# composewell/streamly-lz4

Hardware: AMD Instinct MI355X
Metric: GB/s uncompressed (compress+decompress), 64 KiB blocks, 1/2/4/8 GPU (higher is better)
Workload: dtype u8

## Files before the change

### streamly-lz4_amd/csrc/decode_par.hpp

```cpp
#pragma once

#include "decode_seq.hpp"

namespace lz4dev {

#define PAR_NODES 512
#ifndef PAR_ADAPT
#define PAR_ADAPT 1
#endif
#ifndef PAR_TAIL_ROUND
#define PAR_TAIL_ROUND 2
#endif
#ifndef PAR_ADAPT6
#define PAR_ADAPT6 416
#endif
#ifndef PAR_ADAPT10
#define PAR_ADAPT10 0
#endif
#define PAR_MAXNODES (PAR_ADAPT10 ? 640 : 512)
#ifndef PAR_SQ
#define PAR_SQ 3
#endif
#ifndef PAR_WIN
#define PAR_WIN 832
#endif
#ifndef PAR_RING
#define PAR_RING 5088
#endif
#ifndef PAR_HIST
#define PAR_HIST 1500
#endif
#ifndef PAR_BATCH_OUT
#define PAR_BATCH_OUT 1856
#endif
#ifndef PAR_FAR_WIDE
#define PAR_FAR_WIDE 0
#endif
#ifndef PAR_RANK
#define PAR_RANK 1
#endif
#ifndef PAR_PRIO
#define PAR_PRIO 0x33
#endif
#ifndef PAR_WAVES
#define PAR_WAVES 5
#endif
#ifndef PAR_WAVES_MAIN
#define PAR_WAVES_MAIN 8
#endif

#define PAR_JUMP_BYTES (2 * (PAR_MAXNODES + 8))
#define PAR_JUMP_OFS ((PAR_RING + 32 - PAR_JUMP_BYTES) & ~15)
#define PAR_WIN_BYTES (PAR_WIN + 32)
#define PAR_WIN_OFS (PAR_JUMP_OFS - PAR_WIN_BYTES)
#define PAR_FREE_OFS ((PAR_RING - PAR_BATCH_OUT - 32 + 15) & ~15)
struct __attribute__((aligned(16))) ParLds {
    uint8_t ring[PAR_RING + 32];
    __device__ __forceinline__ uint16_t *jump() { return (uint16_t *)&ring[PAR_JUMP_OFS]; }
    __device__ __forceinline__ uint8_t *win() { return &ring[PAR_WIN_OFS]; }
};
#define PAR_END (2 * PAR_NODES)
#ifndef PAR_LDS_LIMIT
#define PAR_LDS_LIMIT 5120
#endif
static_assert(sizeof(ParLds) <= PAR_LDS_LIMIT, "ParLds above four 1280-byte LDS granules: 24 waves per CU or fewer instead of 28");
static_assert(PAR_WIN_BYTES % 16 == 0 && PAR_JUMP_OFS % 16 == 0 && PAR_WIN_OFS % 16 == 0,
              "the table, its 16-byte rank records and the window's 16-byte slots are aligned");
static_assert(PAR_WIN_OFS >= 0 && PAR_WIN_OFS + PAR_WIN_BYTES <= PAR_JUMP_OFS && PAR_JUMP_OFS + PAR_JUMP_BYTES <= PAR_RING + 32,
              "the window and the table lie inside ring[], one behind the other");
static_assert(PAR_JUMP_BYTES + PAR_WIN_BYTES <= PAR_BATCH_OUT + 64 && PAR_WIN_OFS >= PAR_FREE_OFS && PAR_JUMP_OFS >= PAR_FREE_OFS,
              "the overlays lie on ring bytes that hold no output from a batch's end to the next batch's first store (the no-slide bound)");
#define PAR_WIN_LANES (PAR_WIN / 16)
static_assert(PAR_WIN % 16 == 0 && PAR_WIN_LANES <= LZ4_WAVE, "the window is 16 bytes per lane");
static_assert(PAR_MAXNODES + 288 <= PAR_WIN + 32, "a plain sequence that starts at the last node, and the reads behind it, stay in the window");
static_assert(PAR_HIST + 30 + PAR_BATCH_OUT + 32 <= PAR_RING, "a batch fits the ring right after a slide");

typedef uint64_t par_u64u __attribute__((aligned(1)));
typedef uint32_t par_u32u __attribute__((aligned(1)));
typedef uint16_t par_u16u __attribute__((aligned(1)));

typedef uint32_t par_v4 __attribute__((ext_vector_type(4)));
typedef par_v4 par_v4u __attribute__((aligned(1)));

__device__ __forceinline__ uint32_t lds_u32_any(const uint8_t *base4, uint32_t addr)
{
    const uint32_t *p = (const uint32_t *)(base4 + (addr & ~3u));
    return __builtin_amdgcn_alignbyte(p[1], p[0], addr & 3u);
}
__device__ __forceinline__ uint64_t lds_u64_any(const uint8_t *base4, uint32_t addr)
{
    const uint32_t *p = (const uint32_t *)(base4 + (addr & ~3u));
    const uint32_t d0 = p[0], d1 = p[1], d2 = p[2];
    const uint32_t sh = addr & 3u;
    return ((uint64_t)__builtin_amdgcn_alignbyte(d2, d1, sh) << 32) | __builtin_amdgcn_alignbyte(d1, d0, sh);
}

__device__ __forceinline__ int par_bperm(int v, int srcLane)
{
    return __builtin_amdgcn_ds_bpermute(srcLane << 2, v);
}

template <int D>
__device__ __forceinline__ int par_row_shr(int v)
{
    return __builtin_amdgcn_update_dpp(0, v, 0x110 | D, 0xf, 0xf, true);
}

__device__ __forceinline__ int par_scan_incl(int x)
{
    x += __builtin_amdgcn_update_dpp(0, x, 0x111, 0xf, 0xf, true);
    x += __builtin_amdgcn_update_dpp(0, x, 0x112, 0xf, 0xf, true);
    x += __builtin_amdgcn_update_dpp(0, x, 0x114, 0xf, 0xf, true);
    x += __builtin_amdgcn_update_dpp(0, x, 0x118, 0xf, 0xf, true);
    x += __builtin_amdgcn_update_dpp(0, x, 0x142, 0xa, 0xf, false);
    x += __builtin_amdgcn_update_dpp(0, x, 0x143, 0xc, 0xf, false);
    return x;
}

__device__ __forceinline__ uint4 par_fetch_window_edge(const uint8_t *q, const uint8_t *bufLo, const uint8_t *bufHi)
{
    uint32_t E[8] = {0u, 0u, 0u, 0u, 0u, 0u, 0u, 0u};
    uint32_t m = 0;
    if (q + 16 > bufLo && q < bufHi) {
        const uint8_t *qc = (q < bufLo) ? bufLo : bufHi - 16;
        par_v4 v;
        __builtin_memcpy(&v, as_global(qc), 16);
        const bool below = q < bufLo;
        const uint32_t d = (uint32_t)(below ? bufLo - q : q - qc);
        m = below ? 16u - d : d;
        E[0] = below ? 0u : v.x; E[1] = below ? 0u : v.y; E[2] = below ? 0u : v.z; E[3] = below ? 0u : v.w;
        E[4] = below ? v.x : 0u; E[5] = below ? v.y : 0u; E[6] = below ? v.z : 0u; E[7] = below ? v.w : 0u;
    }
    if (m & 8u) { for (int i = 0; i < 6; i++) E[i] = E[i + 2]; }
    if (m & 4u) { for (int i = 0; i < 5; i++) E[i] = E[i + 1]; }
    uint32_t w[4];
    for (int i = 0; i < 4; i++) w[i] = __builtin_amdgcn_alignbyte(E[i + 1], E[i], m & 3u);
    return make_uint4(w[0], w[1], w[2], w[3]);
}

enum { PS_BATCHES, PS_SEQS, PS_ROUNDS, PS_MATCH_ITERS, PS_LIT_ITERS, PS_HANDOVERS, PS_SLIDES, PS_FULL, PS_FAR,
       PS_T_WINDOW, PS_T_SPEC, PS_T_CHAIN, PS_T_DECODE, PS_T_LIT, PS_T_NEED, PS_T_MATCH, PS_T_FLUSH, PS_T_SEQ, PS_COUNT };

template <bool STATS, bool DICT, bool TOL = false, bool LIST = false, bool PARTIAL = false>
__device__ int decode_block_par(const uint8_t *src, int srcLen, uint8_t *dst, int cap, const uint8_t *dict,
                                uint32_t dictLen, const uint8_t *bufLo, const uint8_t *bufHi, ParLds &L,
                                unsigned long long *stats, TolCtx *tol = nullptr, const uint8_t *list = nullptr,
                                int listLen = 0)
{
    int li = 0;
    int nodesPerLane = 8;
    uint32_t sc[PS_COUNT];
    uint32_t tmark = 0;
    if (STATS) {
#pragma unroll
        for (int i = 0; i < PS_COUNT; i++) sc[i] = 0;
        tmark = (uint32_t)__builtin_amdgcn_readfirstlane((int)(uint32_t)__builtin_amdgcn_s_memtime());
    }
    auto lap = [&](int which) {
        if (STATS) {
            const uint32_t now = (uint32_t)__builtin_amdgcn_readfirstlane((int)(uint32_t)__builtin_amdgcn_s_memtime());
            sc[which] += now - tmark;
            tmark = now;
        }
    };
    auto publish = [&]() {
        if (STATS && lane_id() == 0) {
#pragma unroll
            for (int i = 0; i < PS_COUNT; i++) atomicAdd(&stats[i], (unsigned long long)sc[i]);
        }
    };
    static_assert(!PARTIAL || (!DICT && !TOL), "the partial mode has no dictionary");
    if (DICT) {
        auto up = [](const uint8_t *p) -> const uint8_t * { return (const uint8_t *)(uintptr_t)uni64((int64_t)(uintptr_t)p); };
        src = up(src); dst = (uint8_t *)up(dst); dict = up(dict); bufLo = up(bufLo); bufHi = up(bufHi); list = up(list);
        srcLen = uni(srcLen); cap = uni(cap); dictLen = (uint32_t)uni((int)dictLen); listLen = uni(listLen);
    }
    if (cap < 128 || srcLen < 64) return decode_block_seq<TOL, PARTIAL>(src, srcLen, dst, cap, dict, dictLen, bufLo, bufHi, tol);
    if (!DICT) { dict = nullptr; dictLen = 0; }
    const uint8_t *dictEnd = DICT ? dict + dictLen : dst;
    const int dictLo = DICT ? -(int)min(dictLen, 65535u) : 0;

    int lane;
    asm volatile("v_mbcnt_lo_u32_b32 %0, -1, 0\n\tv_mbcnt_hi_u32_b32 %0, -1, %0" : "=v"(lane));
    const int iend = srcLen;
    const uint32_t A = (uint32_t)((uintptr_t)dst & 15);
    int ip = 0, op = 0;
    int ringBase = 0;
    int flushed = 0;
    SeqState st;

    auto fresh = [](int v) -> int { asm volatile("" : "+v"(v)); return v; };
    constexpr bool MAIN = !DICT && !TOL && !PARTIAL;
    auto win_lane = [&]() -> int { return (PAR_WIN_LANES < LZ4_WAVE) ? min(lane, PAR_WIN_LANES - 1) : lane; };
    auto fetch_window = [&](uintptr_t base) -> uint4 {
        const uint8_t *q = (const uint8_t *)(base + 16u * (uint32_t)win_lane());
        if (__builtin_expect(q >= bufLo && q + 16 <= bufHi, 1)) {
            const par_v4 v = *as_global((const par_v4 *)q);
            return make_uint4(v.x, v.y, v.z, v.w);
        }
        return par_fetch_window_edge(q, bufLo, bufHi);
    };

#ifndef PAR_FLUSH
#define PAR_FLUSH 64
#endif
    const uint32_t AF = (uint32_t)((uintptr_t)dst & (PAR_FLUSH - 1));
    auto flush = [&](int upto, bool final) {
        wave_fence();
        int f = flushed;
        const int mis = (int)((AF + (uint32_t)f) & (PAR_FLUSH - 1));
        if (mis) {
            const int head = PAR_FLUSH - mis;
            if (upto - f >= head) {
                if (lane < head) dst[f + lane] = L.ring[f - ringBase + (int)A + lane];
                f += head;
            } else if (!final) {
                return;
            }
        }
        if (((AF + (uint32_t)f) & (PAR_FLUSH - 1)) == 0) {
            const int n16 = final ? (upto - f) >> 4 : ((upto - f) / PAR_FLUSH) * (PAR_FLUSH / 16);
            for (int c = fresh(lane); c < n16; c += LZ4_WAVE) {
                const uint4 v = *(const uint4 *)&L.ring[f - ringBase + (int)A + 16 * c];
                *(uint4 *)(dst + f + 16 * c) = v;
            }
            f += n16 << 4;
        }
        if (final) {
            for (int x = f + lane; x < upto; x += LZ4_WAVE) dst[x] = L.ring[x - ringBase + (int)A];
            f = upto;
        }
        flushed = f;
        wave_fence();
    };

    uintptr_t wbase = (uintptr_t)src & ~(uintptr_t)15;
    uint4 wnext = fetch_window(wbase);
    bool winStale = true;
    const uint8_t *jumpB = (const uint8_t *)L.jump();

    for (;;) {
        while (iend - ip >= 64 && cap - op >= 128) {
            lap(PS_T_FLUSH);

            const uint8_t *gp = src + ip;
            const uintptr_t abase = (uintptr_t)gp & ~(uintptr_t)15;
            const int wofs = (int)((uintptr_t)gp - abase);
            const int ipW0 = ip - wofs;
            const int iendW = iend - ipW0;
            const int inLim = min(iendW - 32, PAR_WIN);
            if (abase != wbase) { wbase = abase; wnext = fetch_window(abase); winStale = true; }
            if (winStale) {
                *(uint4 *)&L.win()[16 * win_lane()] = wnext;
                winStale = false;
                wave_fence();
            }
            lap(PS_T_WINDOW);

            uint32_t c2, absorb;
            bool fromList = false;
            if (LIST && li < listLen) {
                fromList = true;
                absorb = 2u * (uint32_t)max(inLim, 0);
                const int k = li + lane;
                const uint32_t d = (k < listLen) ? (uint32_t)as_global(list)[k] : 0u;
                const uint64_t zm = __ballot(d == 0u);
                const int known = zm ? (int)__builtin_ctzll(zm) : LZ4_WAVE - 1;
                const int incl0 = par_scan_incl((int)d);
                c2 = (lane <= known) ? 2u * (uint32_t)(wofs + incl0 - (int)d) : absorb;
                c2 = min(c2, absorb);
            } else {
            const int &laneId = lane;
            auto parse_square = [&](auto NC) {
                constexpr int NL = decltype(NC)::value;
                static_assert(NL % 2 == 0 && NL * LZ4_WAVE <= PAR_MAXNODES, "pairs of nodes, table size");
                const int lane = MAIN ? fresh(laneId) : laneId;
                uint32_t J[NL];
                absorb = 2u * ((uint32_t)min(inLim, NL * LZ4_WAVE - 1) + 1u);
                {
                    typedef unsigned short par_h2 __attribute__((ext_vector_type(2)));
                    uint32_t w0, w1, w2;
                    if (NL == 8) {
                        const uint64_t lo = *(const uint64_t *)&L.win()[8 * lane];
                        w0 = (uint32_t)lo; w1 = (uint32_t)(lo >> 32);
                        w2 = (uint32_t)__builtin_amdgcn_update_dpp(0, (int)w0, 0x130, 0xf, 0xf, false);
                    } else {
                        const uint32_t a = (uint32_t)(NL * lane);
                        const uint32_t *q = (const uint32_t *)&L.win()[a & ~3u];
                        const uint32_t d0 = q[0], d1 = q[1], d2 = q[2], d3 = q[3];
                        const uint32_t sh = a & 3u;
                        w0 = __builtin_amdgcn_alignbyte(d1, d0, sh);
                        w1 = __builtin_amdgcn_alignbyte(d2, d1, sh);
                        w2 = __builtin_amdgcn_alignbyte(d3, d2, sh);
                    }
                    auto h2 = [](uint32_t x) { par_h2 r; __builtin_memcpy(&r, &x, 4); return r; };
                    auto u32 = [](par_h2 x) { uint32_t r; __builtin_memcpy(&r, &x, 4); return r; };
                    const par_h2 one = {1, 1}, lim = h2((absorb >> 1) * 0x00010001u);
                    const uint32_t base3 = ((uint32_t)(NL * lane) + 3u) * 0x00010001u + 0x00010000u;
                    uint32_t P[NL / 2];
#pragma unroll
                    for (int p = 0; p < NL / 2; p++) {
                        const uint32_t ws = (p < 2) ? w0 : ((p < 4) ? w1 : w2), wn = (p < 2) ? w1 : w2;
                        const par_h2 T = h2(__builtin_amdgcn_perm(0u, ws, (p & 1) ? 0x0c030c02u : 0x0c010c00u));
                        const par_h2 B = h2((p & 1) ? __builtin_amdgcn_perm(wn, ws, 0x0c040c03u) : __builtin_amdgcn_perm(0u, ws, 0x0c020c01u));
                        const par_h2 lit0 = T >> 4;
                        const par_h2 ext = (lit0 + one) >> 4;
                        const par_h2 term = ext * (B + one) + lit0;
                        const par_h2 mlx = ((T & (par_h2){15, 15}) + one) >> 4;
                        const par_h2 nxt = term + mlx + h2(base3 + 0x00020002u * (uint32_t)p);
                        P[p] = u32(__builtin_elementwise_min(nxt, lim) << 1);
                    }
                    uint32_t *tw = (uint32_t *)&L.jump()[NL * lane];
#pragma unroll
                    for (int p = 0; p < NL / 2; p++) tw[p] = P[p];
                    if (lane == 0) L.jump()[NL * LZ4_WAVE + lane] = (uint16_t)(2 * NL * LZ4_WAVE);
#pragma unroll
                    for (int p = 0; p < NL / 2; p++) { J[2 * p] = P[p] & 0xffffu; J[2 * p + 1] = P[p] >> 16; }
                }
                wave_fence();
                lap(PS_T_SPEC);
#if PAR_PRIO
            if ((PAR_PRIO >> 0 & 3) != (PAR_PRIO >> 6 & 3)) __builtin_amdgcn_s_setprio(PAR_PRIO >> 0 & 3);
#endif

                c2 = (lane == 0) ? 2u * (uint32_t)wofs : absorb;
#pragma unroll
                for (int k = 0; k < PAR_SQ; k++) {
                    const int d = 1 << k;
                    const int cj = (int)*(const uint16_t *)(jumpB + c2);
#pragma unroll
                    for (int j = 0; j < NL; j++) J[j] = (uint32_t)*(const uint16_t *)(jumpB + J[j]);
                    int sh;
                    if (k == 0) sh = par_row_shr<1>(cj);
                    else if (k == 1) sh = par_row_shr<2>(cj);
                    else if (k == 2) sh = par_row_shr<4>(cj);
                    else sh = par_row_shr<8>(cj);
                    if (lane >= d && lane < 2 * d) c2 = (uint32_t)sh;
                    wave_fence();
                    uint32_t *tw = (uint32_t *)&L.jump()[NL * lane];
#pragma unroll
                    for (int p = 0; p < NL / 2; p++) tw[p] = J[2 * p] | (J[2 * p + 1] << 16);
                    wave_fence();
                }
            };
#ifdef PAR_FORCE_NL
            parse_square(std::integral_constant<int, PAR_FORCE_NL>());
#elif PAR_ADAPT
            if (nodesPerLane == 6) parse_square(std::integral_constant<int, 6>());
#if PAR_ADAPT10
            else if (nodesPerLane == 10) parse_square(std::integral_constant<int, 10>());
#endif
            else
                parse_square(std::integral_constant<int, 8>());
#else
                parse_square(std::integral_constant<int, 8>());
#endif
            {
                constexpr int G = 1 << PAR_SQ;
#pragma unroll
                for (int g = 1; g < LZ4_WAVE / G; g++) {
                    int cj = (int)absorb;
                    if (lane >= G * (g - 1) && lane < G * g) cj = (int)*(const uint16_t *)(jumpB + c2);
                    int sh;
                    if (G == 1 && (g & 15)) sh = par_row_shr<1>(cj);
                    else if (G == 2 && (g & 7)) sh = par_row_shr<2>(cj);
                    else if (G == 4 && (g & 3)) sh = par_row_shr<4>(cj);
                    else if (G == 8 && (g & 1)) sh = par_row_shr<8>(cj);
#ifndef PAR_GROUP_BPERM
                    else if (G == 8 && (g == 2 || g == 6)) {
                        const auto r = __builtin_amdgcn_permlane16_swap((unsigned)cj, (unsigned)cj, false, false);
                        sh = __builtin_amdgcn_update_dpp(0, (int)r[0], 0x128 , 0xf, 0xf, false);
                    } else if (G == 8 && g == 4) {
                        const auto q = __builtin_amdgcn_permlane32_swap((unsigned)cj, (unsigned)cj, false, false);
                        const auto r = __builtin_amdgcn_permlane16_swap(q[0], q[0], false, false);
                        sh = __builtin_amdgcn_update_dpp(0, (int)r[1], 0x128 , 0xf, 0xf, false);
                    }
#endif
                    else sh = par_bperm(cj, (lane - G) & 63);
                    if (lane >= G * g && lane < G * g + G) c2 = (uint32_t)sh;
                }
            }
            }
            lap(PS_T_CHAIN);
#if PAR_PRIO
            if ((PAR_PRIO >> 2 & 3) != (PAR_PRIO >> 0 & 3)) __builtin_amdgcn_s_setprio(PAR_PRIO >> 2 & 3);
#endif

            const bool has = c2 < absorb;
            const uint32_t cc = has ? (c2 >> 1) : 0u;
            const uint32_t tb = lds_u32_any(L.win(), cc);
            const uint32_t t = tb & 0xffu, b1 = (tb >> 8) & 0xffu;
            const bool is15 = (t >> 4) == 15u;
            const uint32_t lit = is15 ? 15u + b1 : (t >> 4);
            const uint32_t litStart = cc + 1u + (is15 ? 1u : 0u);
            const uint32_t offPos = litStart + lit;
            const uint32_t ob = lds_u32_any(L.win(), offPos);
            const uint32_t off16 = ob & 0xffffu, b2 = (ob >> 16) & 0xffu;
            const bool mlx = (t & 15u) == 15u;
            const uint32_t ml = (t & 15u) + LZ4_MINMATCH + (mlx ? b2 : 0u);
            const uint32_t nxt = offPos + 2u + (mlx ? 1u : 0u);
            bool ok = has && !(is15 && b1 == 255u) && !(mlx && b2 == 255u) && (int)nxt <= inLim && off16 != 0;
            bool listBad = false;
            if (LIST && fromList) {
                const uint32_t prevNxt = (uint32_t)__builtin_amdgcn_update_dpp(0, (int)nxt, 0x138 , 0xf, 0xf, false);
                listBad = has && lane > 0 && prevNxt != cc;
                ok = ok && !listBad;
            }
            const int len = ok ? (int)(lit + ml) : 0;
            const int incl = par_scan_incl(len);
            const int outEnd = op + incl;
            const int outStart = outEnd - len;
            const int dpos = outStart + (int)lit;
            const int spos = dpos - (int)off16;
            ok = ok && incl <= PAR_BATCH_OUT && outEnd + 64 < cap &&
                 ((spos >= 0 && (spos >= ringBase || spos + (int)ml <= flushed)) ||
                  (DICT && spos >= dictLo && spos + (int)ml <= 0 && (!PAR_FAR_WIDE || ml >= 16u || spos + 16 <= 0)) ||
                  (TOL && spos < 0));
            const uint64_t okm = __ballot(ok);
            const int nseq = (~okm) ? (int)__builtin_ctzll(~okm) : LZ4_WAVE;
            if (LIST && fromList) {
                if (nseq < LZ4_WAVE && ((__ballot(listBad) >> nseq) & 1ull)) listLen = 0;
                li += nseq;
            }
            lap(PS_T_DECODE);
            if (STATS) { sc[PS_BATCHES]++; sc[PS_SEQS] += (unsigned)nseq; if (nseq == LZ4_WAVE) sc[PS_FULL]++; }
            if (nseq == 0) break;

            const bool act = lane < nseq;
            const int opNext = __builtin_amdgcn_readlane(outEnd, nseq - 1);
            const int ipNext = ipW0 + __builtin_amdgcn_readlane((int)nxt, nseq - 1);
            if (PAR_ADAPT && !fromList && nseq >= 16) {
                const int need = (ipNext - ip) * LZ4_WAVE;
                nodesPerLane = (need <= PAR_ADAPT6 * nseq) ? 6 : ((need <= 520 * nseq || !PAR_ADAPT10) ? 8 : 10);
            } else if (PAR_ADAPT && !fromList && nodesPerLane == 6 && !((__ballot(has) >> nseq) & 1ull)) {
                nodesPerLane = 8;
            }
            const uint32_t mdA = (uint32_t)(dpos - ringBase) + A;
            const bool ext = TOL && spos < 0;
            const bool nearSrc = spos >= ringBase && !ext;
            bool deferred = false;
            const bool w8 = ml >= 8 && off16 >= 8;
            const bool grp = w8 && (off16 >= 32 || off16 >= ml);
            const bool g16 = grp && ml >= 16;
            const bool g8 = grp && ml < 16;
            const bool g4 = ml < 8 && off16 >= ml;
            const bool fastc = g16 || g8 || g4;

            const uint64_t farm = __ballot(act && !nearSrc);
            if (TOL && farm) {
                if (act && !nearSrc && (ext || tol_tainted(tol, spos, spos + (int)ml))) {
                    deferred = true;
                    tol_taint(tol, dpos, dpos + (int)ml);
                }
                wave_fence();
            }
            const uint8_t *gsrcD = (DICT && spos < 0) ? dictEnd + spos : dst + spos;
            auto gsrc_at = [&](uint32_t k) -> const uint8_t * { return DICT ? gsrcD + k : dst + (size_t)((uint32_t)spos + k); };
            const bool farMine = act && !nearSrc && !deferred;
            const uint32_t fstep = (ml >= 16) ? 16u : ((ml >= 8) ? 8u : 4u);
            const uint32_t flast = ml - fstep;
            par_v4 f0 = {0u, 0u, 0u, 0u}, f1 = {0u, 0u, 0u, 0u};
            uint64_t fa = 0, fb = 0;
            uint32_t fw0 = 0, fw1 = 0;
            if (farm) {
                if (STATS) sc[PS_FAR] += (unsigned)__builtin_popcountll(farm);
#if PAR_FAR_WIDE
                if (farMine) __builtin_memcpy(&f0, gsrc_at(0u), 16);
                if (farMine && fstep == 16 && ml > 16u) __builtin_memcpy(&f1, gsrc_at(min(16u, flast)), 16);
#else
                if (farMine && fstep == 16) {
                    __builtin_memcpy(&f0, gsrc_at(0u), 16);
                    __builtin_memcpy(&f1, gsrc_at(min(16u, flast)), 16);
                }
                if (farMine && fstep == 8) {
                    fa = *(const par_u64u *)gsrc_at(0u);
                    fb = *(const par_u64u *)gsrc_at(flast);
                }
                if (farMine && fstep == 4) {
                    fw0 = *(const par_u32u *)gsrc_at(0u);
                    fw1 = *(const par_u32u *)gsrc_at(flast);
                }
#endif
            }
            {
                const uintptr_t nb = (uintptr_t)(src + ipNext) & ~(uintptr_t)15;
                wbase = nb;
                wnext = fetch_window(nb);
            }

            uint64_t need = 0;
#if PAR_RANK
            {
                static_assert(16 * (PAR_BATCH_OUT / 64 + 1) <= 2 * PAR_NODES, "rank records fit the jump table");
                uint8_t *rk = (uint8_t *)L.jump();
                constexpr int NREC = PAR_BATCH_OUT / 64 + 1;
                {
                    uint32_t z = 0;
                    asm volatile("" : "+v"(z));
                    if (lane < NREC) *(uint4 *)&rk[16 * lane] = make_uint4(z, z, z, z);
                }
                wave_fence();
                if (act) {
                    const uint32_t rel = (uint32_t)(outStart - op);
                    atomicOr((uint32_t *)&rk[16u * (rel >> 6) + 4u * ((rel >> 5) & 1u)], 1u << (rel & 31u));
                }
                wave_fence();
                {
                    uint2 w = make_uint2(0u, 0u);
                    if (lane < NREC) w = *(const uint2 *)&rk[16 * lane];
                    const int cnt = (int)__builtin_popcount(w.x) + (int)__builtin_popcount(w.y);
                    const int pre = par_scan_incl(cnt) - cnt;
                    if (lane < NREC) *(uint32_t *)&rk[16 * lane + 8] = (uint32_t)pre;
                }
                wave_fence();
                const int srcHi = min(spos + (int)ml, outStart);
                if (act && nearSrc && srcHi > op && srcHi > spos) {
                    const uint32_t xlo = (uint32_t)(max(spos, op) - op), xhi = (uint32_t)(srcHi - 1 - op);
                    auto rank = [&](uint32_t x) -> int {
                        const uint4 r = *(const uint4 *)&rk[16u * (x >> 6)];
                        const uint32_t m = (2u << (x & 31u)) - 1u;
                        const bool hi = (x & 32u) != 0u;
                        return (int)r.z + (int)__builtin_popcount(r.x & (hi ? ~0u : m)) + (int)__builtin_popcount(r.y & (hi ? m : 0u)) - 1;
                    };
                    const int jlo = rank(xlo), jhi = rank(xhi);
                    const uint64_t upto = (jhi >= 63) ? ~0ull : ((1ull << (jhi + 1)) - 1ull);
                    need = upto & ~((1ull << jlo) - 1ull);
                    need &= ~(1ull << fresh(lane));
                }
                wave_fence();
            }
#else
            {
                const int srcHi = min(spos + (int)ml, outStart);
                const int xlo = max(spos, op), xhi = max(srcHi - 1, op);
                int jlo = 0, jhi = 0;
#pragma unroll
                for (int stp = 32; stp >= 1; stp >>= 1) {
                    const int c1 = jlo + stp, cb = jhi + stp;
                    const int v1 = par_bperm(outStart, c1 & 63), v2 = par_bperm(outStart, cb & 63);
                    if (c1 < nseq && v1 <= xlo) jlo = c1;
                    if (cb < nseq && v2 <= xhi) jhi = cb;
                }
                if (act && nearSrc && srcHi > op && srcHi > spos) {
                    const uint64_t upto = (jhi >= 63) ? ~0ull : ((1ull << (jhi + 1)) - 1ull);
                    need = upto & ~((1ull << jlo) - 1ull);
                    need &= ~(1ull << lane);
                }
            }
#endif
            {
                const uint32_t sA = litStart;
                const uint32_t dA = (uint32_t)(outStart - ringBase) + A;
                const uint32_t n = act ? lit : 0u;
                const uint8_t *W = L.win();
                par_v4 r0 = {0u, 0u, 0u, 0u}, r1 = {0u, 0u, 0u, 0u};
                if (n > 8) {
                    if (n + ml >= 16) {
                        r0 = *(const par_v4u *)&W[sA];
                        if (n > 16) r1 = *(const par_v4u *)&W[sA + n - 16];
                    } else {
                        const uint64_t a = *(const par_u64u *)&W[sA], b = *(const par_u64u *)&W[sA + n - 8];
                        r0.x = (uint32_t)a; r0.y = (uint32_t)(a >> 32); r0.z = (uint32_t)b; r0.w = (uint32_t)(b >> 32);
                    }
                } else if (n > 0) {
                    const uint64_t v = lds_u64_any(W, sA);
                    r0.x = (uint32_t)v; r0.y = (uint32_t)(v >> 32);
                }
                wave_fence();
                if (n > 8) {
                    if (n + ml >= 16) {
                        *(par_v4u *)&L.ring[dA] = r0;
                        if (n > 16) {
                            *(par_v4u *)&L.ring[dA + n - 16] = r1;
                            const uint8_t *g = src + ipW0;
                            for (uint32_t o = 16; o < n - 16; o += 16) {
                                par_v4 v;
                                __builtin_memcpy(&v, g + (size_t)(sA + o), 16);
                                *(par_v4u *)&L.ring[dA + o] = v;
                            }
                        }
                    } else {
                        *(par_u64u *)&L.ring[dA] = (uint64_t)r0.x | ((uint64_t)r0.y << 32);
                        *(par_u64u *)&L.ring[dA + n - 8] = (uint64_t)r0.z | ((uint64_t)r0.w << 32);
                    }
                } else if (n > 0) {
                    const uint64_t v = (uint64_t)r0.x | ((uint64_t)r0.y << 32);
                    if (n + ml >= 8) {
                        *(par_u64u *)&L.ring[dA] = v;
                    } else {
                        uint64_t w = v;
                        for (uint32_t q = 0; q < n; q++) { L.ring[dA + q] = (uint8_t)w; w >>= 8; }
                    }
                }
            }
            wave_fence();

            if (farm) {
#if PAR_FAR_WIDE
                if (fstep == 16 && ml <= 16u) f1 = f0;
                {
                    const uint32_t sh = ml - 8u;
                    const bool up = (sh & 4u) != 0u;
                    const uint32_t lo = up ? f0.y : f0.x, mid = up ? f0.z : f0.y, hi = up ? f0.w : f0.z;
                    fa = (uint64_t)f0.x | ((uint64_t)f0.y << 32);
                    fb = (uint64_t)__builtin_amdgcn_alignbyte(mid, lo, sh & 3u) | ((uint64_t)__builtin_amdgcn_alignbyte(hi, mid, sh & 3u) << 32);
                    fw0 = f0.x;
                    fw1 = __builtin_amdgcn_alignbyte(f0.y, f0.x, (ml - 4u) & 3u);
                }
#endif
                if (farMine && fstep == 16) {
                    *(par_v4u *)&L.ring[mdA] = f0;
                    *(par_v4u *)&L.ring[mdA + min(16u, flast)] = f1;
                }
                if (farMine && fstep == 8) {
                    *(par_u64u *)&L.ring[mdA] = fa;
                    *(par_u64u *)&L.ring[mdA + flast] = fb;
                }
                if (farMine && fstep == 4) {
                    *(par_u32u *)&L.ring[mdA] = fw0;
                    *(par_u32u *)&L.ring[mdA + flast] = fw1;
                }
                for (uint32_t base = 32; __ballot(farMine && base < ml); base += 32) {
                    par_v4 v0 = {0u, 0u, 0u, 0u}, v1 = {0u, 0u, 0u, 0u};
                    const bool on = farMine && base < ml;
                    const uint32_t o0 = min(base, flast), o1 = min(base + 16u, flast);
                    if (on) {
                        __builtin_memcpy(&v0, gsrc_at(o0), 16);
                        __builtin_memcpy(&v1, gsrc_at(o1), 16);
                    }
                    if (on) {
                        *(par_v4u *)&L.ring[mdA + o0] = v0;
                        *(par_v4u *)&L.ring[mdA + o1] = v1;
                    }
                }
            }

            lap(PS_T_NEED);
#if PAR_PRIO
            if ((PAR_PRIO >> 4 & 3) != (PAR_PRIO >> 2 & 3)) __builtin_amdgcn_s_setprio(PAR_PRIO >> 4 & 3);
#endif
            need &= ~farm;
            uint64_t done = ((nseq >= LZ4_WAVE) ? 0ull : (~0ull << nseq)) | farm;
            bool pending = act && nearSrc;
            const uint32_t msA = nearSrc ? (uint32_t)(spos - ringBase) + A : 0u;
            int roundNo = 0;
            while (~done) {
#if PAR_TAIL_ROUND
                if (!TOL && roundNo >= PAR_TAIL_ROUND) {
                    for (uint64_t sm = __ballot(pending); sm; sm &= sm - 1) {
                        if (STATS) sc[PS_MATCH_ITERS]++;
                        const int k = (int)__builtin_ctzll(sm);
                        const uint32_t kd = (uint32_t)__builtin_amdgcn_readlane((int)mdA, k);
                        const uint32_t ks = (uint32_t)__builtin_amdgcn_readlane((int)msA, k);
                        const uint32_t koff = (uint32_t)__builtin_amdgcn_readlane((int)off16, k);
                        const uint32_t kml = (uint32_t)__builtin_amdgcn_readlane((int)ml, k);
                        if (koff >= kml) {
                            if ((uint32_t)lane < kml) L.ring[kd + (uint32_t)lane] = L.ring[ks + (uint32_t)lane];
                            for (uint32_t j = (uint32_t)lane + LZ4_WAVE; j < kml; j += LZ4_WAVE) L.ring[kd + j] = L.ring[ks + j];
                        } else {
                            const float rcp = 1.0f / (float)koff;
                            for (uint32_t j = (uint32_t)lane; j < kml; j += LZ4_WAVE) {
                                const uint32_t q = (uint32_t)((float)j * rcp);
                                int rem = (int)j - (int)(q * koff);
                                if (rem < 0) rem += (int)koff; else if (rem >= (int)koff) rem -= (int)koff;
                                L.ring[kd + j] = L.ring[ks + (uint32_t)rem];
                            }
                        }
                        wave_fence();
                    }
                    pending = false;
                    break;
                }
                roundNo++;
#endif
                const bool ready = pending && ((need & ~done) == 0ull);
                bool mine = ready;
                if (TOL) {
                    const int srcHi = min(spos + (int)ml, dpos);
                    if (ready && srcHi > spos && tol_tainted(tol, spos, srcHi)) {
                        deferred = true;
                        mine = false;
                        tol_taint(tol, dpos, dpos + (int)ml);
                    }
                    wave_fence();
                }
                if (STATS) sc[PS_ROUNDS]++;
                for (uint32_t base = 0; __ballot(mine && fastc && base < ml); base += 32) {
                    if (STATS) sc[PS_MATCH_ITERS]++;
                    const bool on = mine && fastc && base < ml;
                    const uint32_t cs = g16 ? 16u : (g8 ? 8u : 4u);
                    const uint32_t lastc = ml - cs;
                    const uint32_t o0 = g16 ? min(base, lastc) : 0u;
                    const uint32_t o1 = g16 ? min(base + 16u, lastc) : lastc;
                    par_v4 v0 = {0u, 0u, 0u, 0u}, v1 = {0u, 0u, 0u, 0u};
                    uint64_t na = 0, nc = 0;
                    uint32_t nw0 = 0, nw1 = 0;
                    if (on) v0 = *(const par_v4u *)&L.ring[msA + o0];
                    if (on && g16 && ml > 16u) v1 = *(const par_v4u *)&L.ring[msA + o1];
                    if (g16 && ml <= 16u) v1 = v0;
                    {
                        const uint32_t sh = ml - 8u;
                        const bool up = (sh & 4u) != 0u;
                        const uint32_t lo = up ? v0.y : v0.x, mid = up ? v0.z : v0.y, hi = up ? v0.w : v0.z;
                        na = (uint64_t)v0.x | ((uint64_t)v0.y << 32);
                        nc = (uint64_t)__builtin_amdgcn_alignbyte(mid, lo, sh & 3u) | ((uint64_t)__builtin_amdgcn_alignbyte(hi, mid, sh & 3u) << 32);
                        nw0 = v0.x;
                        nw1 = __builtin_amdgcn_alignbyte(v0.y, v0.x, (ml - 4u) & 3u);
                    }
                    if (on && g16) {
                        *(par_v4u *)&L.ring[mdA + o0] = v0;
                        *(par_v4u *)&L.ring[mdA + o1] = v1;
                    }
                    if (on && g8) {
                        *(par_u64u *)&L.ring[mdA] = na;
                        *(par_u64u *)&L.ring[mdA + o1] = nc;
                    }
                    if (on && g4) {
                        *(par_u32u *)&L.ring[mdA] = nw0;
                        *(par_u32u *)&L.ring[mdA + o1] = nw1;
                    }
                    wave_fence();
                }
                for (uint64_t sm = __ballot(mine && !fastc); sm; sm &= sm - 1) {
                    if (STATS) sc[PS_MATCH_ITERS]++;
                    const int k = (int)__builtin_ctzll(sm);
                    const uint32_t kd = (uint32_t)__builtin_amdgcn_readlane((int)mdA, k);
                    const uint32_t ks = (uint32_t)__builtin_amdgcn_readlane((int)msA, k);
                    const uint32_t koff = (uint32_t)__builtin_amdgcn_readlane((int)off16, k);
                    const uint32_t kml = (uint32_t)__builtin_amdgcn_readlane((int)ml, k);
                    const float rcp = 1.0f / (float)koff;
                    for (uint32_t j = (uint32_t)lane; j < kml; j += LZ4_WAVE) {
                        const uint32_t q = (uint32_t)((float)j * rcp);
                        int rem = (int)j - (int)(q * koff);
                        if (rem < 0) rem += (int)koff; else if (rem >= (int)koff) rem -= (int)koff;
                        L.ring[kd + j] = L.ring[ks + (uint32_t)rem];
                    }
                    wave_fence();
                }
                pending = pending && !ready;
                done |= __ballot(ready);
            }
            wave_fence();
            if (TOL) {
                const uint64_t dm = __ballot(deferred);
                if (dm) {
                    const uint32_t rank = __builtin_amdgcn_mbcnt_hi((uint32_t)(dm >> 32), __builtin_amdgcn_mbcnt_lo((uint32_t)dm, 0u));
                    const uint32_t base = tol->count;
                    if (deferred && base + rank < tol->cap) tol->list[base + rank] = tol_entry(dpos, spos, ml);
                    wave_fence();
                    if (lane == 0) tol->count = base + (uint32_t)__builtin_popcountll(dm);
                    wave_fence();
                }
            }
            lap(PS_T_MATCH);
#if PAR_PRIO
            if ((PAR_PRIO >> 6 & 3) != (PAR_PRIO >> 4 & 3)) __builtin_amdgcn_s_setprio(PAR_PRIO >> 6 & 3);
#endif

            op = opNext;
            ip = ipNext;
            {
                const par_v4 w = {wnext.x, wnext.y, wnext.z, wnext.w};
                asm volatile("" : : "v"(w));
            }
            flush(op, false);
            if (op - ringBase + (int)A + PAR_BATCH_OUT + 32 > PAR_RING) {
                if (STATS) sc[PS_SLIDES]++;
                const int newBase = (op - PAR_HIST) & ~15;
                const int delta = newBase - ringBase;
                const int n16 = (op - newBase + (int)A + 15) >> 4;
                constexpr int PAR_SLIDE = (PAR_HIST + 45 + 16 * LZ4_WAVE - 1) / (16 * LZ4_WAVE);
                {
                    uint4 v[PAR_SLIDE];
#pragma unroll
                    for (int i = 0; i < PAR_SLIDE; i++) {
                        const int k = lane + i * LZ4_WAVE;
                        v[i] = (k < n16) ? *(const uint4 *)&L.ring[delta + 16 * k] : make_uint4(0u, 0u, 0u, 0u);
                    }
                    wave_fence();
#pragma unroll
                    for (int i = 0; i < PAR_SLIDE; i++) {
                        const int k = lane + i * LZ4_WAVE;
                        if (k < n16) *(uint4 *)&L.ring[16 * k] = v[i];
                    }
                }
                ringBase = newBase;
                wave_fence();
            }
            *(uint4 *)&L.win()[16 * min(fresh(lane), PAR_WIN_LANES - 1)] = wnext;
            wave_fence();
        }

        flush(op, true);
        st.ip = ip; st.op = op; st.fast = true;
        const bool tail = (iend - ip < 64 || cap - op < 128);
        if (STATS && !tail) sc[PS_HANDOVERS]++;
        lap(PS_T_FLUSH);
        if (!DICT && !TOL && !PARTIAL) asm volatile("" : "=v"(lane), "=v"(wnext.x), "=v"(wnext.y), "=v"(wnext.z), "=v"(wnext.w));
        int r = decode_seq_dispatch<TOL, PARTIAL>(st, tail ? 0 : 1, src, srcLen, dst, cap, dict, dictLen, bufLo, bufHi, tol);
        r = uni(r);
        if (r == SEQ_CONTINUE && (!uni((int)st.fast) || iend - uni(st.ip) < 64 || cap - uni(st.op) < 128))
            r = decode_seq_dispatch<TOL, PARTIAL>(st, 0, src, srcLen, dst, cap, dict, dictLen, bufLo, bufHi, tol);
        lap(PS_T_SEQ);
        r = uni(r);
        if (r != SEQ_CONTINUE) { publish(); return r; }
        ip = uni(st.ip); op = uni(st.op);
        if (LIST) li += 1;
        asm volatile("v_mbcnt_lo_u32_b32 %0, -1, 0\n\tv_mbcnt_hi_u32_b32 %0, -1, %0" : "=v"(lane));
        wbase = (uintptr_t)(src + ip) & ~(uintptr_t)15;
        wnext = fetch_window(wbase);
        winStale = true;
        wave_fence();
        ringBase = (op > PAR_HIST) ? ((op - PAR_HIST) & ~15) : 0;
        flushed = op;
        for (int x = ringBase + lane; x < op; x += LZ4_WAVE) L.ring[x - ringBase + (int)A] = dst[x];
        wave_fence();
        lap(PS_T_SEQ);
    }
}

}
```

Measured before the change: 1199.

## Interleave parse node assignment across lanes and store jump table with addtid writes

Reassigns which window positions each lane parses: instead of each lane owning NL consecutive nodes, lane pairs own strided 2-node slices spaced 128 positions apart, read via per-pair word loads and a DPP neighbour exchange. The jump table is then written with ds_write_addtid_b32 (M0-based, lane-indexed stores) through inline asm, or with a strided fallback. The aim is to avoid LDS bank conflicts and unaligned window reads in the speculative parse stage, at the cost of inline asm that saves and restores M0 and assumes a particular table layout.

```diff
diff --git a/streamly-lz4_amd/csrc/decode_par.hpp b/streamly-lz4_amd/csrc/decode_par.hpp
--- a/streamly-lz4_amd/csrc/decode_par.hpp
+++ b/streamly-lz4_amd/csrc/decode_par.hpp
@@ -115,6 +115,37 @@
     x += __builtin_amdgcn_update_dpp(0, x, 0x142, 0xa, 0xf, false);
     x += __builtin_amdgcn_update_dpp(0, x, 0x143, 0xc, 0xf, false);
     return x;
+}
+
+#ifndef PAR_TW
+#define PAR_TW 2
+#endif
+template <int NL, bool TID>
+__device__ __forceinline__ void par_table_store(uint16_t *jump, int lane, const uint32_t (&P)[NL / 2])
+{
+    static_assert(NL == 6 || NL == 8 || NL == 10, "three, four or five pairs");
+    if (PAR_TW == 2 && TID) {
+        const uint32_t jb = (uint32_t)__builtin_amdgcn_readfirstlane((int)(uint32_t)(uintptr_t)jump);
+        const uint32_t p3 = P[NL / 2 > 3 ? 3 : 0], p4 = P[NL / 2 > 4 ? 4 : 0];
+        uint32_t m0keep;
+        if (NL == 6)
+            asm volatile("s_mov_b32 %0, m0\n\ts_mov_b32 m0, %1\n\ts_nop 0\n\tds_write_addtid_b32 %2\n\tds_write_addtid_b32 %3 offset:256\n\t"
+                         "ds_write_addtid_b32 %4 offset:512\n\ts_mov_b32 m0, %0\n\ts_nop 0"
+                         : "=&s"(m0keep) : "s"(jb), "v"(P[0]), "v"(P[1]), "v"(P[2]) : "memory");
+        else if (NL == 8)
+            asm volatile("s_mov_b32 %0, m0\n\ts_mov_b32 m0, %1\n\ts_nop 0\n\tds_write_addtid_b32 %2\n\tds_write_addtid_b32 %3 offset:256\n\t"
+                         "ds_write_addtid_b32 %4 offset:512\n\tds_write_addtid_b32 %5 offset:768\n\ts_mov_b32 m0, %0\n\ts_nop 0"
+                         : "=&s"(m0keep) : "s"(jb), "v"(P[0]), "v"(P[1]), "v"(P[2]), "v"(p3) : "memory");
+        else
+            asm volatile("s_mov_b32 %0, m0\n\ts_mov_b32 m0, %1\n\ts_nop 0\n\tds_write_addtid_b32 %2\n\tds_write_addtid_b32 %3 offset:256\n\t"
+                         "ds_write_addtid_b32 %4 offset:512\n\tds_write_addtid_b32 %5 offset:768\n\tds_write_addtid_b32 %6 offset:1024\n\t"
+                         "s_mov_b32 m0, %0\n\ts_nop 0"
+                         : "=&s"(m0keep) : "s"(jb), "v"(P[0]), "v"(P[1]), "v"(P[2]), "v"(p3), "v"(p4) : "memory");
+    } else {
+        uint32_t *tw = (uint32_t *)&jump[2 * lane];
+#pragma unroll
+        for (int p = 0; p < NL / 2; p++) tw[64 * p] = P[p];
+    }
 }
 
 __device__ __forceinline__ uint4 par_fetch_window_edge(const uint8_t *q, const uint8_t *bufLo, const uint8_t *bufHi)
@@ -279,40 +310,28 @@
                 absorb = 2u * ((uint32_t)min(inLim, NL * LZ4_WAVE - 1) + 1u);
                 {
                     typedef unsigned short par_h2 __attribute__((ext_vector_type(2)));
-                    uint32_t w0, w1, w2;
-                    if (NL == 8) {
-                        const uint64_t lo = *(const uint64_t *)&L.win()[8 * lane];
-                        w0 = (uint32_t)lo; w1 = (uint32_t)(lo >> 32);
-                        w2 = (uint32_t)__builtin_amdgcn_update_dpp(0, (int)w0, 0x130, 0xf, 0xf, false);
-                    } else {
-                        const uint32_t a = (uint32_t)(NL * lane);
-                        const uint32_t *q = (const uint32_t *)&L.win()[a & ~3u];
-                        const uint32_t d0 = q[0], d1 = q[1], d2 = q[2], d3 = q[3];
-                        const uint32_t sh = a & 3u;
-                        w0 = __builtin_amdgcn_alignbyte(d1, d0, sh);
-                        w1 = __builtin_amdgcn_alignbyte(d2, d1, sh);
-                        w2 = __builtin_amdgcn_alignbyte(d3, d2, sh);
-                    }
                     auto h2 = [](uint32_t x) { par_h2 r; __builtin_memcpy(&r, &x, 4); return r; };
                     auto u32 = [](par_h2 x) { uint32_t r; __builtin_memcpy(&r, &x, 4); return r; };
                     const par_h2 one = {1, 1}, lim = h2((absorb >> 1) * 0x00010001u);
-                    const uint32_t base3 = ((uint32_t)(NL * lane) + 3u) * 0x00010001u + 0x00010000u;
+                    const uint32_t *wq = (const uint32_t *)&L.win()[4 * ((lane + 1) >> 1)];
+                    const uint32_t wsh = 2u * ((uint32_t)lane & 1u);
+                    const uint32_t base3 = (2u * (uint32_t)lane + 3u) * 0x00010001u + 0x00010000u;
                     uint32_t P[NL / 2];
 #pragma unroll
                     for (int p = 0; p < NL / 2; p++) {
-                        const uint32_t ws = (p < 2) ? w0 : ((p < 4) ? w1 : w2), wn = (p < 2) ? w1 : w2;
-                        const par_h2 T = h2(__builtin_amdgcn_perm(0u, ws, (p & 1) ? 0x0c030c02u : 0x0c010c00u));
-                        const par_h2 B = h2((p & 1) ? __builtin_amdgcn_perm(wn, ws, 0x0c040c03u) : __builtin_amdgcn_perm(0u, ws, 0x0c020c01u));
+                        const uint32_t dn = wq[32 * p];
+                        const uint32_t de = (uint32_t)__builtin_amdgcn_update_dpp((int)dn, (int)dn, 0xa0 , 0xf, 0xf, false);
+                        const uint32_t ws = __builtin_amdgcn_alignbyte(dn, de, wsh);
+                        const par_h2 T = h2(__builtin_amdgcn_perm(0u, ws, 0x0c010c00u));
+                        const par_h2 B = h2(__builtin_amdgcn_perm(0u, ws, 0x0c020c01u));
                         const par_h2 lit0 = T >> 4;
                         const par_h2 ext = (lit0 + one) >> 4;
                         const par_h2 term = ext * (B + one) + lit0;
                         const par_h2 mlx = ((T & (par_h2){15, 15}) + one) >> 4;
-                        const par_h2 nxt = term + mlx + h2(base3 + 0x00020002u * (uint32_t)p);
+                        const par_h2 nxt = term + mlx + h2(base3 + 0x00800080u * (uint32_t)p);
                         P[p] = u32(__builtin_elementwise_min(nxt, lim) << 1);
                     }
-                    uint32_t *tw = (uint32_t *)&L.jump()[NL * lane];
-#pragma unroll
-                    for (int p = 0; p < NL / 2; p++) tw[p] = P[p];
+                    par_table_store<NL, MAIN>(L.jump(), lane, P);
                     if (lane == 0) L.jump()[NL * LZ4_WAVE + lane] = (uint16_t)(2 * NL * LZ4_WAVE);
 #pragma unroll
                     for (int p = 0; p < NL / 2; p++) { J[2 * p] = P[p] & 0xffffu; J[2 * p + 1] = P[p] >> 16; }
@@ -337,9 +356,10 @@
                     else sh = par_row_shr<8>(cj);
                     if (lane >= d && lane < 2 * d) c2 = (uint32_t)sh;
                     wave_fence();
-                    uint32_t *tw = (uint32_t *)&L.jump()[NL * lane];
-#pragma unroll
-                    for (int p = 0; p < NL / 2; p++) tw[p] = J[2 * p] | (J[2 * p + 1] << 16);
+                    uint32_t P[NL / 2];
+#pragma unroll
+                    for (int p = 0; p < NL / 2; p++) P[p] = J[2 * p] | (J[2 * p + 1] << 16);
+                    par_table_store<NL, MAIN>(L.jump(), lane, P);
                     wave_fence();
                 }
             };
```

Result: faster. 1268 (median of 6 runs) (+5.8%).
